# VISION-SJTU/UniDefense

Measured on AMD Instinct MI355X. Metric: images/sec fwd+bwd (256x256, EffNet-b4), higher is better.
Workload: dtype f32

## Files before the change

### include/unidefense_hip.h

```cpp
#ifndef UNIDEFENSE_HIP_H
#define UNIDEFENSE_HIP_H
#include <stdint.h>

#ifdef __cplusplus
extern "C" {
#endif

#define UD_EINVAL (-1000)

typedef void* ud_stream_t;

typedef struct {
    int N, Hin, Win, Cin, Hout, Wout, KH, KW, stride, pad_t, pad_l, transposed;
} ud_conv_geom;

typedef struct {
    const float* A; const float* B; float* C;
    int M, N, K;
    long lda, ldb, ldc;
    int a_mode, b_mode, out_mode, split_k;
    int batch; long strideA, strideB, strideC;
    ud_conv_geom g;
    double* stat_sum; double* stat_sumsq;
    int half_mask;
// ... 427 lines not shown
                          const uint32_t* skip_absmax, float* out, uint16_t* planes, long panel_stride, long plane_stride,
                          float* inv_scale, int G, int R, int C, uint32_t* absmax, ud_stream_t stream);
int ud_normbwd_sums(const void* x, const void* dy, const float* keep, float inv_keep, const ud_bn_ref* bn, int
    dy_is_dz, int G, int R, int C, double* s1, double* s2, double* s3, double* ws, int f16, ud_stream_t stream);
int ud_normbwd_apply(const void* x, const void* dy, const float* keep, float inv_keep, const ud_bn_ref* bn, int
    dy_is_dz, const double* s1, const double* s2, const double* s1_local, const double* s2_local, int G, int R,
    int C, void* dx, float* dgamma, float* dbeta, int f16, uint32_t* absmax, ud_stream_t stream);
int ud_normbwd_apply_planes(const float* x, const float* dy, const float* keep, float inv_keep, const ud_bn_ref* bn,
                            int dy_is_dz, const double* s1, const double* s2, const double* s1_local,
                            const double* s2_local, const double* energy, int G, int R, int C, uint16_t* planes,
                            long panel_stride, long plane_stride, float* inv_scale, float* dgamma, float* dbeta,
                            ud_stream_t stream);
int ud_pw_bwd_fused_ok(int CE, int CIN);
int ud_pw_bwd_set_form(int form);
long ud_pw_bwd_fused_grid(long M);
int ud_pw_bwd_fused(const float* e, const float* dz, const ud_bn_ref* bn, const double* s1, const double* s2,
                    const double* s1_local, const double* s2_local, const float* x, const float* w, const float* add, long M,
                    int CE, int CIN, float* dx, float* dw, float* part, float* dgamma, float* dbeta, ud_stream_t stream);
int ud_pj_bwd_fused_ok(int CE, int CO, int HW);
int ud_pj_fwd_fused_ok(int CE, int CO, int HW);
int ud_pj_fwd_fused(const float* d, const ud_bn_ref* bn, const float* s, const float* w, int N, int HW, int CE, int CO, float* p,
                    double* sum, double* sumsq, ud_stream_t stream);
long ud_pj_bwd_fused_grid(int N, int HW, int CE, int CO);
int ud_mb_eval_dw_ok(int Ci, int CE, int K, int stride);
long ud_mb_eval_dw_tiles(int Ho, int Wo, int stride);
int ud_mb_eval_dw(const float* x, const float* we, const ud_bn_ref* bn0, const float* wt, const ud_bn_ref* bn1, float* d, float* part,
                  int N, int H, int W, int Ci, int CE, int Ho, int Wo, int K, int stride, int pad_t, int pad_l, int out_act,
                  ud_stream_t stream);
int ud_mb_eval_dw_h_ok(int Ci, int CE, int K, int stride);
long ud_mb_eval_dw_h_tiles(int Ho, int Wo, int stride);
// ... 135 lines not shown
```

### unidefense_amd/csrc/pjbwd.hip

```cpp
#include "pw_common.h"

#include <type_traits>

namespace {

using namespace pw;

constexpr int NTH = 256;
constexpr int R = 32;

__device__ __forceinline__ void atomic_add_f64(double* p, double v) { unsafeAtomicAdd(p, v); }

template <int CE, int CO, int CC = CE> struct PjCfg {
    static_assert(CE % CC == 0 && CC % 8 == 0 && (CC % 16 == 0 || CC == CE) && CO % 8 == 0 && CO > 16 && CO <= 64, "thin project convs");
    static constexpr int CCP = (CC + 15) / 16 * 16;
    static constexpr int NCH = CE / CC;
    static constexpr int QT = CE / 4;
    static constexpr int Q = CC / 4;
    static constexpr int NIT = (R * Q + NTH - 1) / NTH;
    static constexpr int RI = (NIT * NTH + Q - 1) / Q;
    static constexpr int NBC = CCP / 16;
    static constexpr int NBW = (NBC + 3) / 4;
    static constexpr int CS = CCP * 2 + 16;
    static constexpr int CP = RI * CS;
// ... 656 lines not shown
            for (int c = tid; c < CC; c += NTH) atomic_add_f64(a.energy + c0 + c, eacc[c]);
        }
        acc = ud_wave_sum_d(acc);
        if (lane == 0) wsum[wave] = acc;
        __syncthreads();
        if (tid == 0) atomic_add_f64(a.dalpha + (blockIdx.x & 63), (wsum[0] + wsum[1]) + (wsum[2] + wsum[3]));
    }
}

template <int CE, int CO> struct PjFwdCfg {
    using B = PjCfg<CE, CO>;
    static constexpr int KD = (CE + 31) / 32 * 32;
    static constexpr int KS = KD / 32;
    static constexpr int CS = KD * 2 + 16;
    static constexpr int CP = B::RI * CS;
    static constexpr int LDS = 3 * CP + B::COEF + CE * 4 + 2 * 4 * 32 * 8;
};

struct PjFwdArgs {
    const float* d;
    const float* w;
    const float* s;
    float* p;
    double* sum;
    double* sumsq;
    const double* bsum;
    const double* bsumsq;
    const float* rmean;
    const float* rvar;
    const float* gamma;
    const float* beta;
    double inv_count;
    float eps;
    int act;
    int HW;
    long M;
    long tiles;
};

template <int CE, int CO>
__global__ __launch_bounds__(NTH, 2) void pj_fwd_kernel(PjFwdArgs a) {
    using CB = PjCfg<CE, CO>;
    using CF = PjFwdCfg<CE, CO>;
    static_assert(CO > 16 && CO <= 32, "two 16-column blocks: one (row block, column block) per wave");
    extern __shared__ __attribute__((aligned(16))) char L[];
    char* cimg = L;
    float* coef = reinterpret_cast<float*>(L + 3 * CF::CP);
    float* gate = coef + 4 * CE;
    double* wsum = reinterpret_cast<double*>(gate + CE);
    const lds_char* Lp = (const lds_char*)L;
    const int tid = threadIdx.x, lane = tid & 63;
    const int wave = __builtin_amdgcn_readfirstlane(tid >> 6);
    const int u = lane & 15, g = lane >> 4;
    const int mb = wave >> 1, nb = wave & 1;
    const bool swish = a.act == 1;

    if constexpr (CF::KD != CE) {
        for (int i = tid; i < 3 * CF::CP / 16; i += NTH) reinterpret_cast<u32x4*>(L)[i] = u32x4{0u, 0u, 0u, 0u};
    }
    const f32x4* d4 = reinterpret_cast<const f32x4*>(a.d);
    const long t0 = (long)blockIdx.x * a.tiles / gridDim.x, t1 = (long)(blockIdx.x + 1) * a.tiles / gridDim.x;
    f32x4 rd[CB::NIT];
    auto prefetch = [&](long tile_) {
        const long tile = min(tile_, a.tiles - 1);
        const f32x4* db = d4 + tile * (R * CB::Q);
#pragma unroll
        for (int it = 0; it < CB::NIT; ++it) {
            const int idx = tid + it * NTH;
            rd[it] = db[((it + 1) * NTH <= R * CB::Q || idx < R * CB::Q) ? idx : 0];
// ... 29 lines not shown
            cur_n = n;
            __syncthreads();
        }
#pragma unroll
        for (int it = 0; it < CB::NIT; ++it) {
            const int idx = tid + it * NTH;
            const int row = idx / CB::Q, q = idx - row * CB::Q;
            const f32x4 mu = c4[q], is = c4[CB::Q + q], ga = c4[2 * CB::Q + q], be = c4[3 * CB::Q + q], gt = g4[q];
            f32x4 cv;
#pragma unroll
            for (int k = 0; k < 4; ++k) cv[k] = act_sel(ga[k] * ((rd[it][k] - mu[k]) * is[k]) + be[k], swish) * gt[k];
            store_split4(cimg + row * CF::CS + q * 8, CF::CP, cv);
        }
        __syncthreads();
        prefetch(tile + 1);
        f32x4 acc = {0.f, 0.f, 0.f, 0.f};
        const lds_char* arow = Lp + (16 * mb + u) * CF::CS + g * 16;
#pragma unroll
        for (int ks = 0; ks < CF::KS; ++ks) acc = mma6(read_rows(arow + ks * 64, CF::CP), frag_of(wf[ks]), acc);
        float* po = a.p + (tile * R + 16 * mb + 4 * g) * CO + 16 * nb + u;
        float t1_ = 0.f, t2_ = 0.f;
#pragma unroll
        for (int r = 0; r < 4; ++r) {
            if (CO == 32 || 16 * nb + u < CO) po[r * CO] = acc[r];
            t1_ += acc[r];
            t2_ += acc[r] * acc[r];
        }
        s1 += (double)t1_;
        s2 += (double)t2_;
        __syncthreads();
    }
    if (a.sum) {
        s1 += __shfl_xor(s1, 16, 64); s1 += __shfl_xor(s1, 32, 64);
        s2 += __shfl_xor(s2, 16, 64); s2 += __shfl_xor(s2, 32, 64);
        if (g == 0) { wsum[wave * 16 + u] = s1; wsum[64 + wave * 16 + u] = s2; }
        __syncthreads();
        if (tid < CO) {
            const int nbb = tid >> 4, uu = tid & 15;
            atomic_add_f64(a.sum + tid, wsum[nbb * 16 + uu] + wsum[(2 + nbb) * 16 + uu]);
            atomic_add_f64(a.sumsq + tid, wsum[64 + nbb * 16 + uu] + wsum[64 + (2 + nbb) * 16 + uu]);
        }
    }
}

template <int CE, int CO>
int launch_f(const PjFwdArgs& a, int grid, hipStream_t s) {
    using CF = PjFwdCfg<CE, CO>;
    static_assert(CF::LDS <= 64 * 1024, "dynamic LDS within the default limit");
    hipLaunchKernelGGL((pj_fwd_kernel<CE, CO>), dim3((unsigned)grid), dim3(NTH), CF::LDS, s, a);
    return 0;
}

template <int CE, int CO, int CC, bool SE = false>
int launch_a(const PjArgs& a, int grid, hipStream_t s) {
    using CF = PjCfg<CE, CO, CC>;
    static_assert(CF::LDS_A <= 80 * 1024, "two workgroups per CU");
    static bool attr_set = false;
    if (!attr_set) {
        if (hipFuncSetAttribute(reinterpret_cast<const void*>(&pj_bwd_a_kernel<CE, CO, CC, SE>), hipFuncAttributeMaxDynamicSharedMemorySize,
                                CF::LDS_A) != hipSuccess)
            return UD_EINVAL;
        attr_set = true;
    }
// ... 48 lines not shown
               const float* dgamma, const float* dbeta) {
    return args_ok(d, dp, bn, s, w, N, HW, CE, CO) && ud_pj_bwd_fused_se_ok(CE, CO, HW) && dpool && s1 && s2 && dd &&
           !((dgamma || dbeta) && (!s1_local || !s2_local));
}
void fill_c(PjArgs& a, const float* dpool, float inv_hw, const double* s1, const double* s2, const double* s1_local,
            const double* s2_local, float* dd, float* dgamma, float* dbeta) {
    a.dpool = dpool; a.inv_hw = inv_hw; a.bs1 = s1; a.bs2 = s2; a.bs1l = s1_local; a.bs2l = s2_local; a.dd = dd; a.dgamma = dgamma;
    a.dbeta = dbeta;
}

}

extern "C" {

int ud_pj_bwd_fused_ok(int CE, int CO, int HW) { return (chunk_of(CE, CO) && HW >= R && HW % R == 0) ? 1 : 0; }
int ud_pj_fwd_fused_ok(int CE, int CO, int HW) { return (CO <= 32 && chunk_of(CE, CO) == CE && HW >= R && HW % R == 0) ? 1 : 0; }

int ud_pj_bwd_fused_se_ok(int CE, int CO, int HW) { return (ud_pj_bwd_fused_ok(CE, CO, HW) && CO != 24) ? 1 : 0; }

long ud_pj_bwd_fused_grid(int N, int HW, int CE, int CO) {
    const int cc = chunk_of(CE, CO);
    if (N < 1 || HW < R || HW % R || !cc) return UD_EINVAL;
    const long tiles = (long)N * HW / R, nch = CE / cc, per = 512 / nch;
    return nch * (tiles < per ? tiles : per);
}

int ud_pj_fwd_fused(const float* d, const ud_bn_ref* bn, const float* s, const float* w, int N, int HW, int CE, int CO, float* p,
                     double* sum, double* sumsq, ud_stream_t stream) {
    if (!d || !bn || (!bn->sum && !ud_bn_eval_form(bn)) || !s || !w || !p || N < 1 || !ud_pj_fwd_fused_ok(CE, CO, HW) || bn->G != 1 || !bn->gamma || !bn->beta || (!sum != !sumsq))
        return UD_EINVAL;
    PjFwdArgs a;
    a.d = d; a.w = w; a.s = s; a.p = p; a.sum = sum; a.sumsq = sumsq;
    a.bsum = bn->sum; a.bsumsq = bn->sumsq; a.rmean = bn->running_mean; a.rvar = bn->running_var; a.gamma = bn->gamma; a.beta = bn->beta;
    a.inv_count = bn->inv_count; a.eps = bn->eps; a.act = bn->act; a.HW = HW;
    a.M = (long)N * HW; a.tiles = a.M / R;
    const int grid = (int)ud_pj_bwd_fused_grid(N, HW, CE, CO);
    hipStream_t st = (hipStream_t)stream;
    const int rc = CO == 32 ? (CE == 144 ? launch_f<144, 32>(a, grid, st) : launch_f<192, 32>(a, grid, st))
                            : (CE == 48 ? launch_f<48, 24>(a, grid, st) : launch_f<24, 24>(a, grid, st));
    if (rc) return rc;
    UD_LAUNCH_CHECK();
    return 0;
}

int ud_pj_bwd_fused_a(const float* d, const float* dp, const ud_bn_ref* bn, const float* s, const float* w, int N, int HW, int CE, int CO,
                      float* dw, double* dgate, float* part, ud_stream_t stream) {
    if (!args_ok(d, dp, bn, s, w, N, HW, CE, CO) || !dw || !dgate || !part) return UD_EINVAL;
    hipStream_t st = (hipStream_t)stream;
    PjArgs a;
    fill(a, d, dp, bn, s, w, N, HW, CE, CO);
    a.part = part; a.dgate = dgate;
    const int grid = (int)ud_pj_bwd_fused_grid(N, HW, CE, CO);
    const int rc = CO == 32 ? (CE == 144 ? launch_a<144, 32, 144>(a, grid, st) : launch_a<192, 32, 192>(a, grid, st))
// ... 73 lines not shown
```

### unidefense_amd/csrc/pwbwd.hip

```cpp
#include "pw_common.h"

#include <type_traits>

namespace {

constexpr int NTH = 256;
constexpr int R = 32;

using namespace pw;

template <int CE, int CIN> struct PwCfg {
    static_assert(CE % 16 == 0 && CIN % 8 == 0 && CIN > 16 && CIN <= 32, "thin expand convs: 16 < CIN <= 32");
    static constexpr int KD = (CE + 31) / 32 * 32;
    static constexpr int KS = KD / 32;
    static constexpr int DYS = KD * 2 + 16;
    static constexpr int Q = CE / 4;
    static constexpr int NIT = (R * Q + NTH - 1) / NTH;
    static constexpr int RI = (NIT * NTH + Q - 1) / Q;
    static constexpr int DYP = RI * DYS;
    static constexpr int NB = 2;
    static constexpr int XS = NB * 32 + 16;
    static constexpr int XP = (NTH / (CIN / 4) + 1) * XS;
    static constexpr int XQ = CIN / 4;
    static constexpr int MB = CE / 16;
    static constexpr int NBW = (MB + 1) / 2;
    static constexpr int IMG = 3 * DYP + 3 * XP;
    static constexpr int LDS = IMG + 5 * CE * 4;
};

struct PwArgs {
    const float* e;
    const float* dz;
    const float* x;
    const float* w;
    const float* add;
    float* dx;
    float* part;
    const double* bsum;
    const double* bsumsq;
    const float* gamma;
// ... 2 lines not shown
    double inv_count;
    float eps;
    long M;
    long tiles;
};

template <int CE, int CIN, int D, int WPC>
__global__ __launch_bounds__(NTH, WPC) void pw_bwd_kernel(PwArgs a) {
    using CF = PwCfg<CE, CIN>;
    extern __shared__ __attribute__((aligned(16))) char L[];
    const lds_char* Lp = (const lds_char*)L;
    float* coef = reinterpret_cast<float*>(L + CF::IMG);
    const int tid = threadIdx.x, lane = tid & 63;
    const int wave = __builtin_amdgcn_readfirstlane(tid >> 6);
    const int u = lane & 15, g = lane >> 4;
    const int mb_d = wave >> 1, nbk = wave & 1;

    for (int i = tid; i < CF::IMG / 16; i += NTH) reinterpret_cast<u32x4*>(L)[i] = u32x4{0u, 0u, 0u, 0u};
    for (int c = tid; c < CE; c += NTH) {
        const double m = a.bsum[c] * a.inv_count;
        double v = a.bsumsq[c] * a.inv_count - m * m;
        if (v < 0.0) v = 0.0;
        const float is = rsqrtf((float)(v + (double)a.eps));
        coef[c] = (float)m;
        coef[CE + c] = is;
        coef[2 * CE + c] = a.gamma[c] * is;
        coef[3 * CE + c] = (float)a.s1[c] * (float)a.inv_count;
        coef[4 * CE + c] = (float)a.s2[c] * (float)a.inv_count;
    }

    u32x4 wf[CF::KS][3];
// ... 13 lines not shown
                uint32_t p0, p1, p2;
                split2(v[2 * h], v[2 * h + 1], p0, p1, p2);
                wf[ks][0][h] = p0; wf[ks][1][h] = p1; wf[ks][2][h] = p2;
            }
        }
    }

    f32x4 accw[CF::NBW];
#pragma unroll
    for (int i = 0; i < CF::NBW; ++i) accw[i] = f32x4{0.f, 0.f, 0.f, 0.f};

    const f32x4* dz4 = reinterpret_cast<const f32x4*>(a.dz);
    const f32x4* e4 = reinterpret_cast<const f32x4*>(a.e);
    const f32x4* x4 = reinterpret_cast<const f32x4*>(a.x);
    const long lim4 = a.M * CF::Q, limx = a.M * CF::XQ;
    f32x4 rdz[D][CF::NIT], re[D][CF::NIT], rx[D];
    float rav[D][4];
    const float* const add_src = a.add ? a.add : a.dx;
    const bool has_add = a.add != nullptr;
    const int dcol = 16 * nbk + u;
    auto prefetch = [&](auto slot_c, long tile_) {
        constexpr int S = decltype(slot_c)::value;
        const long tile = min(tile_, a.tiles - 1);
        const long b4 = tile * (R * CF::Q);
#pragma unroll
        for (int it = 0; it < CF::NIT; ++it) {
            const int idx = tid + it * NTH;
            long i = b4 + idx;
            i = (idx < R * CF::Q && i < lim4) ? i : 0;
            rdz[S][it] = dz4[i];
            re[S][it] = e4[i];
        }
        long ix = tile * (R * CF::XQ) + tid;
        ix = (tid < R * CF::XQ && ix < limx) ? ix : 0;
        rx[S] = x4[ix];
        const long row0 = tile * R + 16 * mb_d + 4 * g;
#pragma unroll
        for (int r = 0; r < 4; ++r) rav[S][r] = add_src[min(row0 + r, a.M - 1) * CIN + min(dcol, CIN - 1)];
    };

    const f32x4* c4 = reinterpret_cast<const f32x4*>(coef);
    auto step = [&](auto slot_c, long tile) {
        constexpr int S = decltype(slot_c)::value;
        {
            const long b4 = tile * (R * CF::Q);
#pragma unroll
            for (int it = 0; it < CF::NIT; ++it) {
                const int idx = tid + it * NTH;
                {
                    const int row = idx / CF::Q, q = idx - row * CF::Q;
                    const bool ok = b4 + idx < lim4;
                    const f32x4 mu = c4[q], is = c4[CF::Q + q], gi = c4[2 * CF::Q + q], t1 = c4[3 * CF::Q + q], t2 = c4[4 * CF::Q + q];
                    f32x4 o;
#pragma unroll
                    for (int k = 0; k < 4; ++k) {
                        const float xh = (re[S][it][k] - mu[k]) * is[k];
                        o[k] = ok ? gi[k] * (rdz[S][it][k] - t1[k] - xh * t2[k]) : 0.f;
                    }
                    uint32_t p0[2], p1[2], p2[2];
                    split2(o[0], o[1], p0[0], p1[0], p2[0]);
                    split2(o[2], o[3], p0[1], p1[1], p2[1]);
                    char* dst = L + row * CF::DYS + q * 8;
                    *reinterpret_cast<u32x2*>(dst) = u32x2{p0[0], p0[1]};
                    *reinterpret_cast<u32x2*>(dst + CF::DYP) = u32x2{p1[0], p1[1]};
                    *reinterpret_cast<u32x2*>(dst + 2 * CF::DYP) = u32x2{p2[0], p2[1]};
                }
            }
            {
                const int row = tid / CF::XQ, q = tid - row * CF::XQ;
                const bool ok = tile * (R * CF::XQ) + tid < limx;
                uint32_t p0[2], p1[2], p2[2];
                split2(ok ? rx[S][0] : 0.f, ok ? rx[S][1] : 0.f, p0[0], p1[0], p2[0]);
                split2(ok ? rx[S][2] : 0.f, ok ? rx[S][3] : 0.f, p0[1], p1[1], p2[1]);
                char* dst = L + 3 * CF::DYP + row * CF::XS + q * 8;
                *reinterpret_cast<u32x2*>(dst) = u32x2{p0[0], p0[1]};
                *reinterpret_cast<u32x2*>(dst + CF::XP) = u32x2{p1[0], p1[1]};
                *reinterpret_cast<u32x2*>(dst + 2 * CF::XP) = u32x2{p2[0], p2[1]};
            }
        }
        __syncthreads();
        float av[4];
#pragma unroll
        for (int r = 0; r < 4; ++r) av[r] = has_add ? rav[S][r] : 0.f;
        prefetch(slot_c, tile + (long)D * gridDim.x);

        {
            f32x4 acc = {0.f, 0.f, 0.f, 0.f};
            const int col = dcol;
            const long row0 = tile * R + 16 * mb_d + 4 * g;
            const lds_char* arow = Lp + (16 * mb_d + u) * CF::DYS + g * 16;
#pragma unroll
            for (int ks = 0; ks < CF::KS; ++ks) {
                bf16x8 af[3];
#pragma unroll
                for (int p = 0; p < 3; ++p)
                    af[p] = __builtin_bit_cast(bf16x8, *reinterpret_cast<const __attribute__((address_space(3))) s16x8*>(arow + p * CF::DYP + ks * 64));
                const bf16x8 b0 = __builtin_bit_cast(bf16x8, wf[ks][0]), b1 = __builtin_bit_cast(bf16x8, wf[ks][1]),
                             b2 = __builtin_bit_cast(bf16x8, wf[ks][2]);
                acc = __builtin_amdgcn_mfma_f32_16x16x32_bf16(af[2], b0, acc, 0, 0, 0);
                acc = __builtin_amdgcn_mfma_f32_16x16x32_bf16(af[0], b2, acc, 0, 0, 0);
                acc = __builtin_amdgcn_mfma_f32_16x16x32_bf16(af[1], b1, acc, 0, 0, 0);
                acc = __builtin_amdgcn_mfma_f32_16x16x32_bf16(af[1], b0, acc, 0, 0, 0);
                acc = __builtin_amdgcn_mfma_f32_16x16x32_bf16(af[0], b1, acc, 0, 0, 0);
                acc = __builtin_amdgcn_mfma_f32_16x16x32_bf16(af[0], b0, acc, 0, 0, 0);
            }
#pragma unroll
            for (int r = 0; r < 4; ++r)
                if (col < CIN && row0 + r < a.M) a.dx[(row0 + r) * CIN + col] = acc[r] + av[r];
        }
        {
            const int q = u >> 2, pp = u & 3;
            bf16x8 bf[3];
            const lds_char* xb = Lp + 3 * CF::DYP + (8 * g + q) * CF::XS + (16 * nbk + 4 * pp) * 2;
#pragma unroll
            for (int p = 0; p < 3; ++p) {
                const s16x4 lo = __builtin_amdgcn_ds_read_tr16_b64_v4i16((__attribute__((address_space(3))) s16x4*)(xb + p * CF::XP));
                const s16x4 hi = __builtin_amdgcn_ds_read_tr16_b64_v4i16((__attribute__((address_space(3))) s16x4*)(xb + p * CF::XP + 4 * CF::XS));
                bf[p] = __builtin_bit_cast(bf16x8, __builtin_shufflevector(lo, hi, 0, 1, 2, 3, 4, 5, 6, 7));
            }
            const lds_char* ab = Lp + (8 * g + q) * CF::DYS + 4 * pp * 2;
#pragma unroll
            for (int i = 0; i < CF::NBW; ++i) {
                const int mbk = min((wave >> 1) + 2 * i, CF::MB - 1);
                {
                    bf16x8 af[3];
#pragma unroll
                    for (int p = 0; p < 3; ++p) {
                        const lds_char* s = ab + p * CF::DYP + mbk * 32;
                        const s16x4 lo = __builtin_amdgcn_ds_read_tr16_b64_v4i16((__attribute__((address_space(3))) s16x4*)(s));
                        const s16x4 hi = __builtin_amdgcn_ds_read_tr16_b64_v4i16((__attribute__((address_space(3))) s16x4*)(s + 4 * CF::DYS));
                        af[p] = __builtin_bit_cast(bf16x8, __builtin_shufflevector(lo, hi, 0, 1, 2, 3, 4, 5, 6, 7));
                    }
                    f32x4 c = accw[i];
                    c = __builtin_amdgcn_mfma_f32_16x16x32_bf16(af[2], bf[0], c, 0, 0, 0);
                    c = __builtin_amdgcn_mfma_f32_16x16x32_bf16(af[0], bf[2], c, 0, 0, 0);
                    c = __builtin_amdgcn_mfma_f32_16x16x32_bf16(af[1], bf[1], c, 0, 0, 0);
                    c = __builtin_amdgcn_mfma_f32_16x16x32_bf16(af[1], bf[0], c, 0, 0, 0);
                    c = __builtin_amdgcn_mfma_f32_16x16x32_bf16(af[0], bf[1], c, 0, 0, 0);
                    c = __builtin_amdgcn_mfma_f32_16x16x32_bf16(af[0], bf[0], c, 0, 0, 0);
                    accw[i] = c;
                }
            }
        }
        __syncthreads();
    };

    using std::integral_constant;
    {
        long t = blockIdx.x;
        prefetch(integral_constant<int, 0>{}, t);
        if constexpr (D > 1) { t += gridDim.x; prefetch(integral_constant<int, 1>{}, t); }
        if constexpr (D > 2) { t += gridDim.x; prefetch(integral_constant<int, 2>{}, t); }
        if constexpr (D > 3) { t += gridDim.x; prefetch(integral_constant<int, 3>{}, t); }
    }
    __syncthreads();
    for (long tile = blockIdx.x;;) {
// ... 11 lines not shown
            tile += gridDim.x;
        }
        if constexpr (D > 3) {
            if (tile >= a.tiles) break;
            step(integral_constant<int, 3>{}, tile);
            tile += gridDim.x;
        }
    }

    {
        float* part = a.part + (long)blockIdx.x * (CE * CIN);
        const int col = 16 * nbk + u;
        if (col < CIN) {
#pragma unroll
            for (int i = 0; i < CF::NBW; ++i) {
                const int mbk = (wave >> 1) + 2 * i;
                if (mbk < CF::MB) {
#pragma unroll
                    for (int r = 0; r < 4; ++r) part[(16 * mbk + 4 * g + r) * CIN + col] = accw[i][r];
                }
            }
        }
    }
}

__global__ __launch_bounds__(256) void pw_bwd_fold_kernel(const float* __restrict__ part, int nparts, int numel, float* __restrict__ dw,
                                                          const double* __restrict__ s1l, const double* __restrict__ s2l, int CE,
                                                          float* __restrict__ dgamma, float* __restrict__ dbeta) {
    __shared__ float red[16][17];
    const int el = threadIdx.x & 15, grp = threadIdx.x >> 4;
    const int i = blockIdx.x * 16 + el;
// ... 12 lines not shown
        float t = red[0][el];
#pragma unroll
        for (int j = 1; j < 16; ++j) t += red[j][el];
        dw[i] = t;
    }
    const int c = blockIdx.x * 256 + threadIdx.x;
    if (c < CE) {
        if (dbeta) dbeta[c] = (float)s1l[c];
        if (dgamma) dgamma[c] = (float)s2l[c];
    }
}

template <int CE, int CIN, int D, int WPC>
int launch(const PwArgs& a, int grid, hipStream_t s) {
    using CF = PwCfg<CE, CIN>;
    static_assert(CF::LDS <= 64 * 1024, "dynamic LDS within the default limit");
    hipLaunchKernelGGL((pw_bwd_kernel<CE, CIN, D, WPC>), dim3((unsigned)grid), dim3(NTH), CF::LDS, s, a);
    return 0;
}

int g_pw_form = 0;

}

int pw::fold_launch(const float* part, int nparts, int numel, float* dw, const double* s1l, const double* s2l, int CE, float* dgamma,
                    float* dbeta, hipStream_t s) {
    hipLaunchKernelGGL(pw_bwd_fold_kernel, dim3((unsigned)ud_cdiv(numel, 16)), dim3(256), 0, s, part, nparts, numel, dw, s1l, s2l, CE,
                       dgamma, dbeta);
    UD_LAUNCH_CHECK();
    return 0;
}

extern "C" {

int ud_pw_bwd_set_form(int form) {
    if (form < 0 || form > 4) return UD_EINVAL;
    g_pw_form = form;
    return 0;
}

int ud_pw_bwd_fused_ok(int CE, int CIN) { return (CE == 144 && CIN == 24) || (CE == 192 && CIN == 32); }

long ud_pw_bwd_fused_grid(long M) {
    if (M < 1) return UD_EINVAL;
    const long tiles = (M + R - 1) / R;
    return tiles < 512 ? tiles : 512;
}

int ud_pw_bwd_fused(const float* e, const float* dz, const ud_bn_ref* bn, const double* s1, const double* s2, const double* s1_local,
                    const double* s2_local, const float* x, const float* w, const float* add, long M, int CE, int CIN, float* dx,
                    float* dw, float* part, float* dgamma, float* dbeta, ud_stream_t stream) {
    if (ud_bn_eval_form(bn)) return UD_EINVAL;
    if (!e || !dz || !bn || !s1 || !s2 || !x || !w || !dx || !dw || !part || M < 1 || !ud_pw_bwd_fused_ok(CE, CIN) || bn->G != 1 ||
        !bn->gamma)
        return UD_EINVAL;
    if ((dgamma || dbeta) && (!s1_local || !s2_local)) return UD_EINVAL;
    hipStream_t s = (hipStream_t)stream;
    PwArgs a;
    a.e = e; a.dz = dz; a.x = x; a.w = w; a.add = add; a.dx = dx; a.part = part;
    a.bsum = bn->sum; a.bsumsq = bn->sumsq; a.gamma = bn->gamma; a.s1 = s1; a.s2 = s2;
    a.inv_count = bn->inv_count; a.eps = bn->eps; a.M = M; a.tiles = (M + R - 1) / R;
    const int grid = (int)ud_pw_bwd_fused_grid(M);
    const int form = g_pw_form ? g_pw_form : 1;
    int rc;
    if (CE == 144)
        rc = form == 1 ? launch<144, 24, 1, 2>(a, grid, s) : form == 2 ? launch<144, 24, 2, 2>(a, grid, s)
           : form == 3 ? launch<144, 24, 3, 1>(a, grid, s) : launch<144, 24, 4, 1>(a, grid, s);
    else
        rc = form == 1 ? launch<192, 32, 1, 2>(a, grid, s) : form == 2 ? launch<192, 32, 2, 2>(a, grid, s)
           : form == 3 ? launch<192, 32, 3, 1>(a, grid, s) : launch<192, 32, 4, 1>(a, grid, s);
    if (rc) return rc;
    UD_LAUNCH_CHECK();
    return pw::fold_launch(part, grid, CE * CIN, dw, s1_local, s2_local, CE, dgamma, dbeta, s);
}

}
```

### unidefense_amd/kernels.py

```python
import ctypes as C
import math
import os

import torch

from . import lib as _lib
from .config import cfg as CFG
from .devmem import Scratch, ZeroPool
from .lib import ConvGeom, GemmDesc, GemmP3Desc

_call = _lib.call
_const, _rows = _lib.const, _lib.const_rows

GEMM_PROFILE = None


def _stream():
    return C.c_void_p(torch.cuda.current_stream().cuda_stream)


def _p(t):
    if t is None:
        return None
    return C.c_void_p(t.data_ptr())
# ... 3011 lines not shown


def expand_bwd_fused(e, dz, bn, sacc, sacc_local, x2, w2, add=None):
    _chk(e, dz, x2, w2)
    Ce, Cin = w2.shape
    M = x2.shape[0]
    assert e.numel() == M * Ce and dz.numel() == M * Ce and x2.is_contiguous() and w2.is_contiguous()
    loc = sacc if sacc_local is None else sacc_local
    dx = add if add is not None else torch.empty_like(x2)
    if add is not None:
        _chk(add)
        assert add.numel() == M * Cin
    dw = empty((Ce, Cin), x2)
    dg = empty((Ce,), x2)
    db = empty((Ce,), x2)
    grid = _lib.call("ud_pw_bwd_fused_grid", M)
    part = empty((grid, Ce * Cin), x2)
    _call("ud_pw_bwd_fused", _p(e), _p(dz), C.byref(bn.ref()), _pd(sacc), _pd(sacc, Ce), _pd(loc), _pd(loc, Ce), _p(x2), _p(w2),
          _p(add), M, Ce, Cin, _p(dx), _p(dw), _p(part), _p(dg), _p(db), _stream())
    return dx, dw, dg, db


def project_bwd_fused_ok(d, w2, HW):
    return (CFG.project_bwd_fused and d.dtype == torch.float32 and w2.dtype == torch.float32 and
            (CFG.project_bwd_fused_wide or w2.shape[0] != 56) and (CFG.project_fused_narrow or w2.shape[0] != 24) and
            _lib.call("ud_pj_bwd_fused_ok", int(w2.shape[1]), int(w2.shape[0]), int(HW)) == 1)


def project_fwd_fused_ok(d, w2, HW):
    return (project_bwd_fused_ok(d, w2, HW) and _lib.call("ud_pj_fwd_fused_ok", int(w2.shape[1]), int(w2.shape[0]), int(HW)) == 1)

# ... 467 lines not shown
```

### unidefense_amd/mbconv.py

```python
import collections
from types import SimpleNamespace

import torch

from . import kernels as K
from . import tape as T
from .config import cfg


FUSED, HALF, EVAL_NODE, OPERATORS = "fused", "half", "eval_node", "operators"
TrunkMode = collections.namedtuple("TrunkMode", "kind wt dp", defaults=(None,))


_DW_TILED = True


_DW_TILE_OVERRIDE = {}
_DW_BWD_FUSED_OVERRIDE = {}


def _dw_tile_policy(sf, k, stride, H, half):
    ov = _DW_TILE_OVERRIDE.get((bool(sf), k, stride, H, bool(half)))
    if ov is not None and _DW_TILED:
        return ov
# ... 37 lines not shown
    if ov is not None:
        return ov
    return True


_PJ_BN1_FOLD_OVERRIDE = {}
_PJ_BN1_FOLD_RULE = {(False, 2, 64, 144): True, (False, 1, 64, 192): True, (True, 2, 32, 192): True, (True, 1, 32, 336): True}


def _pj_bn1_fold_policy(sf, stride, Ho, Ce):
    key = (bool(sf), stride, Ho, Ce)
    ov = _PJ_BN1_FOLD_OVERRIDE.get(key)
    if ov is not None:
        return ov
    return _PJ_BN1_FOLD_RULE.get(key, False)


BlockGeom = collections.namedtuple(
    "BlockGeom", "N H W Cin M k stride pt pl Ho Wo HWo Mo Ce Co Cs We Wsr Wse Wp Wf sf alpha s_f s_i")


def block_geom(blk, x):
    sp = blk.spec
    N, H, W, Cin = x.shape
    Ho, Wo = T.conv_out_hw(H, W, sp.k, sp.stride, sp.pad)
    Ce, Co, Cs = sp.cexp, sp.cout, sp.cse
    sf = sp.sf_norm is not None
    dwm = blk._depthwise_conv
    s_f, s_i = T._fft_scales(H, sp.sf_norm) if sf else (None, None)
    return BlockGeom(N, H, W, Cin, N * H * W, sp.k, sp.stride, sp.pad[2], sp.pad[0], Ho, Wo, Ho * Wo, N * Ho * Wo, Ce, Co, Cs,
# ... 183 lines not shown
    b.c_pl = (d.dtype == torch.float32 and g.Ce % 32 == 0 and cfg.spectral_p2 != "off"
              and K.spectral_takes_planes(g.Mo, g.Co, g.Ce, g.Wp, want_stats=True))
    c_amax = None
    if b.c_pl:
        c_amax = K.colsum_bn_amax(d, b.bn1, g.N, g.HWo, b.pool, update=True)
    else:
        K.colsum_bn(d, b.bn1, g.N, g.HWo, b.pool, update=True)
    b.s1 = K.fc_fwd_d(b.pool, 1.0 / g.HWo, g.Wsr, blk._se_reduce.bias, g.N)
    b.s2 = K.fc_fwd(b.s1, g.Wse, blk._se_expand.bias, 1)
    return c_amax


def _fwd_project(b, c_amax, next_blk):
    g, x, blk, d, bn1, s2 = b.geo, b.x, b.blk, b.d, b.bn1, b.s2
    acc2 = K.zeros64(2 * g.Co, x)
    if not b.c_pl and K.project_fwd_fused_ok(d, g.Wp, g.HWo):
        p, b.pctx = K.project_fwd_fused(d, bn1, s2, g.Wp, g.N, g.HWo, stats=acc2)
        done = True
    elif b.c_pl:
        c = K.se_scale_bn_planes(d, bn1, s2, g.N, g.HWo, c_amax)
        (p, done), b.pctx = K.spectral_fwd(c, g.Wp, stats=acc2)
    elif (d.dtype == torch.float16 and g.Ce % 8 == 0 and K.spectral_takes_plane_half(g.Mo, g.Co, g.Ce)):
        c = K.se_scale_bn_plane_half(d, bn1, s2, g.N, g.HWo)
        (p, done), b.pctx = K.spectral_fwd(c, g.Wp, stats=acc2)
    else:
        c = K.se_scale_bn(d, bn1, s2, g.N, g.HWo, want_absmax=True)
        (p, done), b.pctx = K.spectral_fwd(c.view(g.Mo, g.Ce), g.Wp, stats=acc2, x_absmax=getattr(c, "_ud_absmax", None))
    if not done:
        K.colstats(p, acc2)
    b.dp.reduce(acc2)
    b.bn2 = _bn_of(blk._bn2, acc2, g.Mo * b.dp.world, 0)
# ... 169 lines not shown
        if b.t_bwd:
            gr.dx = K.dwtile_bwd_data(g_sp, wt, k, pt, pl, g.H, g.W, g_alpha, g_mode, add, stride=stride)
        else:
            gr.dx = K.dwconv_bwd_data_ex(g_sp, g_alpha, g_mode, wt, add, k, stride, pt, pl, g.H, g.W)
    if not skip_done:
        gr.dx = K.axpby(gr.dx, 1.0, dout, 1.0, out=gr.dx)


def _bwd_expand(b, tape, gr):
    g, x, blk, e, ectx, dz0, sb0, dout = b.geo, b.x, b.blk, b.e, b.ectx, gr.dz0, gr.sb0, gr.dout
    skip = blk.spec.skip
    if b.lazy_in is not None:
        b.lazy_in.backward(dz0, sb0, gr.is_dz)
        return None
    loc0 = b.dp.reduce(sb0, keep_local=True)
    thin = not gr.de_pl and e is not None and ectx.plans is None and K.expand_bwd_fused_ok(e, ectx.w, gr.is_dz)
    if thin:
        dx, dWe, dg0, db0 = _expand_dgrad(tape, skip, dout, x, lambda acc: K.expand_bwd_fused(e, dz0, b.bn0, sb0, loc0, ectx.x, ectx.w, add=acc))
    else:
        de2, de_amax, dg0, db0 = _normbwd_to_gemm(ectx, gr.de_pl, e, dz0, None, 1.0, b.bn0, gr.is_dz, 1, g.M, sb0, loc0)
    tape.add_param_grad(blk._bn0.weight, dg0)
    tape.add_param_grad(blk._bn0.bias, db0)
    if not thin:
        dx, dWe = _expand_dgrad(tape, skip, dout, x, lambda acc: K.spectral_bwd(ectx, de2, out=acc, dy_absmax=de_amax))
    tape.add_param_grad(blk._expand_conv.weight, dWe)
    return dx


def _half_forward(x, blk, g, wt, src_bn):
    bn1 = K.EvalBN(blk._bn1, 1)
    if g.We is not None:
# ... 99 lines not shown
            dx = K.axpby(dx, 1.0, dout, 1.0, out=dx)
    if probe is not None:
        probe(blk, "dx", dx)
    dx._ud_owned = True
    tape.add_grad(x, dx)


def eval_block_ok(blk, max_cin):
    sp = blk.spec
    return (sp.expand != 1 and sp.sf_norm is None and sp.cin <= max_cin and K.mb_eval_dw_ok(sp.cin, sp.cexp, sp.k, sp.stride))


def mbconv_eval(x, blk, wt):
    g = block_geom(blk, x)
    bn1 = K.EvalBN(blk._bn1, 1)
    pj = K.project_fwd_fused_ok(x, g.Wp, g.HWo)
    d, pool = K.mb_eval_dw(x, g.We, K.EvalBN(blk._bn0, 1), wt, bn1, g.k, g.stride, g.pt, g.pl, g.Ho, g.Wo, out_act=not pj)
    s1 = K.fc_fwd(pool, g.Wsr, blk._se_reduce.bias, 0)
    s2 = K.fc_fwd(s1, g.Wse, blk._se_expand.bias, 1)
    if pj:
        p, _ = K.project_fwd_fused(d, bn1, s2, g.Wp, g.N, g.HWo)
    else:
        p = K.gemm_nt(K.se_scale_fwd(d, s2).view(g.Mo, g.Ce), g.Wp)
    return K.residual_bn(p.view(g.N, g.Ho, g.Wo, g.Co), K.EvalBN(blk._bn2, 0), None, 1.0, x if blk.spec.skip else None, g.N, g.HWo)
```

Measured before the change: 1480.

## Extend fused project-forward and expand-backward kernels to 56-channel stages

```diff
diff --git a/include/unidefense_hip.h b/include/unidefense_hip.h
--- a/include/unidefense_hip.h
+++ b/include/unidefense_hip.h
@@ -465,6 +465,7 @@
 int ud_pw_bwd_fused_ok(int CE, int CIN);
 int ud_pw_bwd_set_form(int form);
 long ud_pw_bwd_fused_grid(long M);
+int ud_pw_bwd_fused_parts(long M, int CE, int CIN);
 int ud_pw_bwd_fused(const float* e, const float* dz, const ud_bn_ref* bn, const double* s1, const double* s2,
                     const double* s1_local, const double* s2_local, const float* x, const float* w, const float* add, long M,
                     int CE, int CIN, float* dx, float* dw, float* part, float* dgamma, float* dbeta, ud_stream_t stream);
diff --git a/unidefense_amd/csrc/pjbwd.hip b/unidefense_amd/csrc/pjbwd.hip
--- a/unidefense_amd/csrc/pjbwd.hip
+++ b/unidefense_amd/csrc/pjbwd.hip
@@ -694,7 +694,8 @@
     static constexpr int KS = KD / 32;
     static constexpr int CS = KD * 2 + 16;
     static constexpr int CP = B::RI * CS;
-    static constexpr int LDS = 3 * CP + B::COEF + CE * 4 + 2 * 4 * 32 * 8;
+    static constexpr int WS = CO > 32 ? 2 * 4 * 16 * 8 : 2 * 4 * 32 * 8;
+    static constexpr int LDS = 3 * CP + B::COEF + CE * 4 + WS;
 };
 
 struct PjFwdArgs {
@@ -722,7 +723,9 @@
 __global__ __launch_bounds__(NTH, 2) void pj_fwd_kernel(PjFwdArgs a) {
     using CB = PjCfg<CE, CO>;
     using CF = PjFwdCfg<CE, CO>;
-    static_assert(CO > 16 && CO <= 32, "two 16-column blocks: one (row block, column block) per wave");
+    static_assert(CO > 16 && CO <= 64, "two 16-column blocks: one (row block, column block) per wave; four: a wave owns a column block");
+    constexpr bool WIDE = CO > 32;
+    constexpr int NMB = WIDE ? 2 : 1;
     extern __shared__ __attribute__((aligned(16))) char L[];
     char* cimg = L;
     float* coef = reinterpret_cast<float*>(L + 3 * CF::CP);
@@ -732,7 +735,7 @@
     const int tid = threadIdx.x, lane = tid & 63;
     const int wave = __builtin_amdgcn_readfirstlane(tid >> 6);
     const int u = lane & 15, g = lane >> 4;
-    const int mb = wave >> 1, nb = wave & 1;
+    const int mb = WIDE ? 0 : wave >> 1, nb = WIDE ? wave : wave & 1;
     const bool swish = a.act == 1;
 
     if constexpr (CF::KD != CE) {
@@ -792,17 +795,26 @@
         }
         __syncthreads();
         prefetch(tile + 1);
-        f32x4 acc = {0.f, 0.f, 0.f, 0.f};
+        f32x4 acc[NMB];
+#pragma unroll
+        for (int i = 0; i < NMB; ++i) acc[i] = f32x4{0.f, 0.f, 0.f, 0.f};
         const lds_char* arow = Lp + (16 * mb + u) * CF::CS + g * 16;
 #pragma unroll
-        for (int ks = 0; ks < CF::KS; ++ks) acc = mma6(read_rows(arow + ks * 64, CF::CP), frag_of(wf[ks]), acc);
+        for (int ks = 0; ks < CF::KS; ++ks) {
+            const Frag3 b = frag_of(wf[ks]);
+#pragma unroll
+            for (int i = 0; i < NMB; ++i) acc[i] = mma6(read_rows(arow + i * 16 * CF::CS + ks * 64, CF::CP), b, acc[i]);
+        }
         float* po = a.p + (tile * R + 16 * mb + 4 * g) * CO + 16 * nb + u;
         float t1_ = 0.f, t2_ = 0.f;
 #pragma unroll
-        for (int r = 0; r < 4; ++r) {
-            if (CO == 32 || 16 * nb + u < CO) po[r * CO] = acc[r];
-            t1_ += acc[r];
-            t2_ += acc[r] * acc[r];
+        for (int i = 0; i < NMB; ++i) {
+#pragma unroll
+            for (int r = 0; r < 4; ++r) {
+                if (CO % 16 == 0 || 16 * nb + u < CO) po[(16 * i + r) * CO] = acc[i][r];
+                t1_ += acc[i][r];
+                t2_ += acc[i][r] * acc[i][r];
+            }
         }
         s1 += (double)t1_;
         s2 += (double)t2_;
@@ -815,8 +827,13 @@
         __syncthreads();
         if (tid < CO) {
             const int nbb = tid >> 4, uu = tid & 15;
-            atomic_add_f64(a.sum + tid, wsum[nbb * 16 + uu] + wsum[(2 + nbb) * 16 + uu]);
-            atomic_add_f64(a.sumsq + tid, wsum[64 + nbb * 16 + uu] + wsum[64 + (2 + nbb) * 16 + uu]);
+            if constexpr (WIDE) {
+                atomic_add_f64(a.sum + tid, wsum[nbb * 16 + uu]);
+                atomic_add_f64(a.sumsq + tid, wsum[64 + nbb * 16 + uu]);
+            } else {
+                atomic_add_f64(a.sum + tid, wsum[nbb * 16 + uu] + wsum[(2 + nbb) * 16 + uu]);
+                atomic_add_f64(a.sumsq + tid, wsum[64 + nbb * 16 + uu] + wsum[64 + (2 + nbb) * 16 + uu]);
+            }
         }
     }
 }
@@ -824,7 +841,16 @@
 template <int CE, int CO>
 int launch_f(const PjFwdArgs& a, int grid, hipStream_t s) {
     using CF = PjFwdCfg<CE, CO>;
-    static_assert(CF::LDS <= 64 * 1024, "dynamic LDS within the default limit");
+    static_assert(CF::LDS <= 80 * 1024, "two workgroups per CU");
+    if constexpr (CF::LDS > 64 * 1024) {
+        static bool attr_set = false;
+        if (!attr_set) {
+            if (hipFuncSetAttribute(reinterpret_cast<const void*>(&pj_fwd_kernel<CE, CO>), hipFuncAttributeMaxDynamicSharedMemorySize,
+                                    CF::LDS) != hipSuccess)
+                return UD_EINVAL;
+            attr_set = true;
+        }
+    }
     hipLaunchKernelGGL((pj_fwd_kernel<CE, CO>), dim3((unsigned)grid), dim3(NTH), CF::LDS, s, a);
     return 0;
 }
@@ -903,7 +929,10 @@
 extern "C" {
 
 int ud_pj_bwd_fused_ok(int CE, int CO, int HW) { return (chunk_of(CE, CO) && HW >= R && HW % R == 0) ? 1 : 0; }
-int ud_pj_fwd_fused_ok(int CE, int CO, int HW) { return (CO <= 32 && chunk_of(CE, CO) == CE && HW >= R && HW % R == 0) ? 1 : 0; }
+int ud_pj_fwd_fused_ok(int CE, int CO, int HW) {
+    const bool pair = (CO <= 32 && chunk_of(CE, CO) == CE) || (CO == 56 && (CE == 192 || CE == 336));
+    return (pair && HW >= R && HW % R == 0) ? 1 : 0;
+}
 
 int ud_pj_bwd_fused_se_ok(int CE, int CO, int HW) { return (ud_pj_bwd_fused_ok(CE, CO, HW) && CO != 24) ? 1 : 0; }
 
@@ -923,9 +952,10 @@
     a.bsum = bn->sum; a.bsumsq = bn->sumsq; a.rmean = bn->running_mean; a.rvar = bn->running_var; a.gamma = bn->gamma; a.beta = bn->beta;
     a.inv_count = bn->inv_count; a.eps = bn->eps; a.act = bn->act; a.HW = HW;
     a.M = (long)N * HW; a.tiles = a.M / R;
-    const int grid = (int)ud_pj_bwd_fused_grid(N, HW, CE, CO);
+    const int grid = (int)(a.tiles < 512 ? a.tiles : 512);
     hipStream_t st = (hipStream_t)stream;
     const int rc = CO == 32 ? (CE == 144 ? launch_f<144, 32>(a, grid, st) : launch_f<192, 32>(a, grid, st))
+                 : CO == 56 ? (CE == 336 ? launch_f<336, 56>(a, grid, st) : launch_f<192, 56>(a, grid, st))
                             : (CE == 48 ? launch_f<48, 24>(a, grid, st) : launch_f<24, 24>(a, grid, st));
     if (rc) return rc;
     UD_LAUNCH_CHECK();
diff --git a/unidefense_amd/csrc/pwbwd.hip b/unidefense_amd/csrc/pwbwd.hip
--- a/unidefense_amd/csrc/pwbwd.hip
+++ b/unidefense_amd/csrc/pwbwd.hip
@@ -10,7 +10,7 @@
 using namespace pw;
 
 template <int CE, int CIN> struct PwCfg {
-    static_assert(CE % 16 == 0 && CIN % 8 == 0 && CIN > 16 && CIN <= 32, "thin expand convs: 16 < CIN <= 32");
+    static_assert(CE % 16 == 0 && CIN % 8 == 0 && CIN > 16 && CIN <= 64, "thin expand convs: 16 < CIN <= 64");
     static constexpr int KD = (CE + 31) / 32 * 32;
     static constexpr int KS = KD / 32;
     static constexpr int DYS = KD * 2 + 16;
@@ -18,12 +18,15 @@
     static constexpr int NIT = (R * Q + NTH - 1) / NTH;
     static constexpr int RI = (NIT * NTH + Q - 1) / Q;
     static constexpr int DYP = RI * DYS;
-    static constexpr int NB = 2;
+    static constexpr int NB = CIN > 32 ? 4 : 2;
+    static constexpr bool WIDE = NB == 4;
+    static constexpr int NMB = WIDE ? 2 : 1;
     static constexpr int XS = NB * 32 + 16;
-    static constexpr int XP = (NTH / (CIN / 4) + 1) * XS;
     static constexpr int XQ = CIN / 4;
+    static constexpr int NITX = (R * XQ + NTH - 1) / NTH;
+    static constexpr int XP = (NITX * NTH / XQ + 1) * XS;
     static constexpr int MB = CE / 16;
-    static constexpr int NBW = (MB + 1) / 2;
+    static constexpr int NBW = WIDE ? MB : (MB + 1) / 2;
     static constexpr int IMG = 3 * DYP + 3 * XP;
     static constexpr int LDS = IMG + 5 * CE * 4;
 };
@@ -56,7 +59,7 @@
     const int tid = threadIdx.x, lane = tid & 63;
     const int wave = __builtin_amdgcn_readfirstlane(tid >> 6);
     const int u = lane & 15, g = lane >> 4;
-    const int mb_d = wave >> 1, nbk = wave & 1;
+    const int mb_d = CF::WIDE ? 0 : wave >> 1, nbk = CF::WIDE ? wave : wave & 1;
 
     for (int i = tid; i < CF::IMG / 16; i += NTH) reinterpret_cast<u32x4*>(L)[i] = u32x4{0u, 0u, 0u, 0u};
     for (int c = tid; c < CE; c += NTH) {
@@ -100,8 +103,8 @@
     const f32x4* e4 = reinterpret_cast<const f32x4*>(a.e);
     const f32x4* x4 = reinterpret_cast<const f32x4*>(a.x);
     const long lim4 = a.M * CF::Q, limx = a.M * CF::XQ;
-    f32x4 rdz[D][CF::NIT], re[D][CF::NIT], rx[D];
-    float rav[D][4];
+    f32x4 rdz[D][CF::NIT], re[D][CF::NIT], rx[D][CF::NITX];
+    float rav[D][4 * CF::NMB];
     const float* const add_src = a.add ? a.add : a.dx;
     const bool has_add = a.add != nullptr;
     const int dcol = 16 * nbk + u;
@@ -117,12 +120,18 @@
             rdz[S][it] = dz4[i];
             re[S][it] = e4[i];
         }
-        long ix = tile * (R * CF::XQ) + tid;
-        ix = (tid < R * CF::XQ && ix < limx) ? ix : 0;
-        rx[S] = x4[ix];
+#pragma unroll
+        for (int it = 0; it < CF::NITX; ++it) {
+            const int idx = tid + it * NTH;
+            long ix = tile * (R * CF::XQ) + idx;
+            ix = (idx < R * CF::XQ && ix < limx) ? ix : 0;
+            rx[S][it] = x4[ix];
+        }
         const long row0 = tile * R + 16 * mb_d + 4 * g;
 #pragma unroll
-        for (int r = 0; r < 4; ++r) rav[S][r] = add_src[min(row0 + r, a.M - 1) * CIN + min(dcol, CIN - 1)];
+        for (int i = 0; i < CF::NMB; ++i)
+#pragma unroll
+            for (int r = 0; r < 4; ++r) rav[S][4 * i + r] = add_src[min(row0 + 16 * i + r, a.M - 1) * CIN + min(dcol, CIN - 1)];
     };
 
     const f32x4* c4 = reinterpret_cast<const f32x4*>(coef);
@@ -152,12 +161,14 @@
                     *reinterpret_cast<u32x2*>(dst + 2 * CF::DYP) = u32x2{p2[0], p2[1]};
                 }
             }
-            {
-                const int row = tid / CF::XQ, q = tid - row * CF::XQ;
-                const bool ok = tile * (R * CF::XQ) + tid < limx;
+#pragma unroll
+            for (int it = 0; it < CF::NITX; ++it) {
+                const int idx = tid + it * NTH;
+                const int row = idx / CF::XQ, q = idx - row * CF::XQ;
+                const bool ok = tile * (R * CF::XQ) + idx < limx;
                 uint32_t p0[2], p1[2], p2[2];
-                split2(ok ? rx[S][0] : 0.f, ok ? rx[S][1] : 0.f, p0[0], p1[0], p2[0]);
-                split2(ok ? rx[S][2] : 0.f, ok ? rx[S][3] : 0.f, p0[1], p1[1], p2[1]);
+                split2(ok ? rx[S][it][0] : 0.f, ok ? rx[S][it][1] : 0.f, p0[0], p1[0], p2[0]);
+                split2(ok ? rx[S][it][2] : 0.f, ok ? rx[S][it][3] : 0.f, p0[1], p1[1], p2[1]);
                 char* dst = L + 3 * CF::DYP + row * CF::XS + q * 8;
                 *reinterpret_cast<u32x2*>(dst) = u32x2{p0[0], p0[1]};
                 *reinterpret_cast<u32x2*>(dst + CF::XP) = u32x2{p1[0], p1[1]};
@@ -165,34 +176,41 @@
             }
         }
         __syncthreads();
-        float av[4];
-#pragma unroll
-        for (int r = 0; r < 4; ++r) av[r] = has_add ? rav[S][r] : 0.f;
+        float av[4 * CF::NMB];
+#pragma unroll
+        for (int r = 0; r < 4 * CF::NMB; ++r) av[r] = has_add ? rav[S][r] : 0.f;
         prefetch(slot_c, tile + (long)D * gridDim.x);
 
         {
-            f32x4 acc = {0.f, 0.f, 0.f, 0.f};
+            f32x4 acc[CF::NMB];
+#pragma unroll
+            for (int i = 0; i < CF::NMB; ++i) acc[i] = f32x4{0.f, 0.f, 0.f, 0.f};
             const int col = dcol;
             const long row0 = tile * R + 16 * mb_d + 4 * g;
             const lds_char* arow = Lp + (16 * mb_d + u) * CF::DYS + g * 16;
 #pragma unroll
             for (int ks = 0; ks < CF::KS; ++ks) {
-                bf16x8 af[3];
-#pragma unroll
-                for (int p = 0; p < 3; ++p)
-                    af[p] = __builtin_bit_cast(bf16x8, *reinterpret_cast<const __attribute__((address_space(3))) s16x8*>(arow + p * CF::DYP + ks * 64));
                 const bf16x8 b0 = __builtin_bit_cast(bf16x8, wf[ks][0]), b1 = __builtin_bit_cast(bf16x8, wf[ks][1]),
                              b2 = __builtin_bit_cast(bf16x8, wf[ks][2]);
-                acc = __builtin_amdgcn_mfma_f32_16x16x32_bf16(af[2], b0, acc, 0, 0, 0);
-                acc = __builtin_amdgcn_mfma_f32_16x16x32_bf16(af[0], b2, acc, 0, 0, 0);
-                acc = __builtin_amdgcn_mfma_f32_16x16x32_bf16(af[1], b1, acc, 0, 0, 0);
-                acc = __builtin_amdgcn_mfma_f32_16x16x32_bf16(af[1], b0, acc, 0, 0, 0);
-                acc = __builtin_amdgcn_mfma_f32_16x16x32_bf16(af[0], b1, acc, 0, 0, 0);
-                acc = __builtin_amdgcn_mfma_f32_16x16x32_bf16(af[0], b0, acc, 0, 0, 0);
-            }
-#pragma unroll
-            for (int r = 0; r < 4; ++r)
-                if (col < CIN && row0 + r < a.M) a.dx[(row0 + r) * CIN + col] = acc[r] + av[r];
+#pragma unroll
+                for (int i = 0; i < CF::NMB; ++i) {
+                    bf16x8 af[3];
+#pragma unroll
+                    for (int p = 0; p < 3; ++p)
+                        af[p] = __builtin_bit_cast(bf16x8, *reinterpret_cast<const __attribute__((address_space(3))) s16x8*>(arow + i * 16 * CF::DYS + p * CF::DYP + ks * 64));
+                    acc[i] = __builtin_amdgcn_mfma_f32_16x16x32_bf16(af[2], b0, acc[i], 0, 0, 0);
+                    acc[i] = __builtin_amdgcn_mfma_f32_16x16x32_bf16(af[0], b2, acc[i], 0, 0, 0);
+                    acc[i] = __builtin_amdgcn_mfma_f32_16x16x32_bf16(af[1], b1, acc[i], 0, 0, 0);
+                    acc[i] = __builtin_amdgcn_mfma_f32_16x16x32_bf16(af[1], b0, acc[i], 0, 0, 0);
+                    acc[i] = __builtin_amdgcn_mfma_f32_16x16x32_bf16(af[0], b1, acc[i], 0, 0, 0);
+                    acc[i] = __builtin_amdgcn_mfma_f32_16x16x32_bf16(af[0], b0, acc[i], 0, 0, 0);
+                }
+            }
+#pragma unroll
+            for (int i = 0; i < CF::NMB; ++i)
+#pragma unroll
+                for (int r = 0; r < 4; ++r)
+                    if (col < CIN && row0 + 16 * i + r < a.M) a.dx[(row0 + 16 * i + r) * CIN + col] = acc[i][r] + av[4 * i + r];
         }
         {
             const int q = u >> 2, pp = u & 3;
@@ -205,27 +223,28 @@
                 bf[p] = __builtin_bit_cast(bf16x8, __builtin_shufflevector(lo, hi, 0, 1, 2, 3, 4, 5, 6, 7));
             }
             const lds_char* ab = Lp + (8 * g + q) * CF::DYS + 4 * pp * 2;
-#pragma unroll
-            for (int i = 0; i < CF::NBW; ++i) {
-                const int mbk = min((wave >> 1) + 2 * i, CF::MB - 1);
-                {
-                    bf16x8 af[3];
+            constexpr int GB = CF::WIDE ? 3 : 1;
+            static_assert(CF::NBW % GB == 0, "whole groups of row blocks");
+#pragma unroll
+            for (int i = 0; i < CF::NBW; i += GB) {
+                bf16x8 af[GB][3];
+#pragma unroll
+                for (int j = 0; j < GB; ++j) {
+                    const int mbk = CF::WIDE ? i + j : min((wave >> 1) + 2 * i, CF::MB - 1);
 #pragma unroll
                     for (int p = 0; p < 3; ++p) {
                         const lds_char* s = ab + p * CF::DYP + mbk * 32;
                         const s16x4 lo = __builtin_amdgcn_ds_read_tr16_b64_v4i16((__attribute__((address_space(3))) s16x4*)(s));
                         const s16x4 hi = __builtin_amdgcn_ds_read_tr16_b64_v4i16((__attribute__((address_space(3))) s16x4*)(s + 4 * CF::DYS));
-                        af[p] = __builtin_bit_cast(bf16x8, __builtin_shufflevector(lo, hi, 0, 1, 2, 3, 4, 5, 6, 7));
+                        af[j][p] = __builtin_bit_cast(bf16x8, __builtin_shufflevector(lo, hi, 0, 1, 2, 3, 4, 5, 6, 7));
                     }
-                    f32x4 c = accw[i];
-                    c = __builtin_amdgcn_mfma_f32_16x16x32_bf16(af[2], bf[0], c, 0, 0, 0);
-                    c = __builtin_amdgcn_mfma_f32_16x16x32_bf16(af[0], bf[2], c, 0, 0, 0);
-                    c = __builtin_amdgcn_mfma_f32_16x16x32_bf16(af[1], bf[1], c, 0, 0, 0);
-                    c = __builtin_amdgcn_mfma_f32_16x16x32_bf16(af[1], bf[0], c, 0, 0, 0);
-                    c = __builtin_amdgcn_mfma_f32_16x16x32_bf16(af[0], bf[1], c, 0, 0, 0);
-                    c = __builtin_amdgcn_mfma_f32_16x16x32_bf16(af[0], bf[0], c, 0, 0, 0);
-                    accw[i] = c;
                 }
+                constexpr int PA[6] = {2, 0, 1, 1, 0, 0}, PB[6] = {0, 2, 1, 0, 1, 0};
+#pragma unroll
+                for (int t = 0; t < 6; ++t)
+#pragma unroll
+                    for (int j = 0; j < GB; ++j)
+                        accw[i + j] = __builtin_amdgcn_mfma_f32_16x16x32_bf16(af[j][PA[t]], bf[PB[t]], accw[i + j], 0, 0, 0);
             }
         }
         __syncthreads();
@@ -267,7 +286,7 @@
         if (col < CIN) {
 #pragma unroll
             for (int i = 0; i < CF::NBW; ++i) {
-                const int mbk = (wave >> 1) + 2 * i;
+                const int mbk = CF::WIDE ? i : (wave >> 1) + 2 * i;
                 if (mbk < CF::MB) {
 #pragma unroll
                     for (int r = 0; r < 4; ++r) part[(16 * mbk + 4 * g + r) * CIN + col] = accw[i][r];
@@ -310,7 +329,16 @@
 template <int CE, int CIN, int D, int WPC>
 int launch(const PwArgs& a, int grid, hipStream_t s) {
     using CF = PwCfg<CE, CIN>;
-    static_assert(CF::LDS <= 64 * 1024, "dynamic LDS within the default limit");
+    static_assert(CF::LDS <= 160 * 1024 / WPC, "WPC workgroups per CU");
+    if constexpr (CF::LDS > 64 * 1024) {
+        static bool attr_set = false;
+        if (!attr_set) {
+            if (hipFuncSetAttribute(reinterpret_cast<const void*>(&pw_bwd_kernel<CE, CIN, D, WPC>), hipFuncAttributeMaxDynamicSharedMemorySize,
+                                    CF::LDS) != hipSuccess)
+                return UD_EINVAL;
+            attr_set = true;
+        }
+    }
     hipLaunchKernelGGL((pw_bwd_kernel<CE, CIN, D, WPC>), dim3((unsigned)grid), dim3(NTH), CF::LDS, s, a);
     return 0;
 }
@@ -335,12 +363,18 @@
     return 0;
 }
 
-int ud_pw_bwd_fused_ok(int CE, int CIN) { return (CE == 144 && CIN == 24) || (CE == 192 && CIN == 32); }
+int ud_pw_bwd_fused_ok(int CE, int CIN) { return (CE == 144 && CIN == 24) || (CE == 192 && CIN == 32) || (CE == 336 && CIN == 56); }
 
 long ud_pw_bwd_fused_grid(long M) {
     if (M < 1) return UD_EINVAL;
     const long tiles = (M + R - 1) / R;
     return tiles < 512 ? tiles : 512;
+}
+
+int ud_pw_bwd_fused_parts(long M, int CE, int CIN) {
+    if (M < 1 || !ud_pw_bwd_fused_ok(CE, CIN)) return UD_EINVAL;
+    const int g = (int)ud_pw_bwd_fused_grid(M);
+    return (CIN > 32 && g > 256) ? 256 : g;
 }
 
 int ud_pw_bwd_fused(const float* e, const float* dz, const ud_bn_ref* bn, const double* s1, const double* s2, const double* s1_local,
@@ -356,10 +390,12 @@
     a.e = e; a.dz = dz; a.x = x; a.w = w; a.add = add; a.dx = dx; a.part = part;
     a.bsum = bn->sum; a.bsumsq = bn->sumsq; a.gamma = bn->gamma; a.s1 = s1; a.s2 = s2;
     a.inv_count = bn->inv_count; a.eps = bn->eps; a.M = M; a.tiles = (M + R - 1) / R;
-    const int grid = (int)ud_pw_bwd_fused_grid(M);
+    const int grid = ud_pw_bwd_fused_parts(M, CE, CIN);
     const int form = g_pw_form ? g_pw_form : 1;
     int rc;
-    if (CE == 144)
+    if (CE == 336)
+        rc = launch<336, 56, 1, 1>(a, grid, s);
+    else if (CE == 144)
         rc = form == 1 ? launch<144, 24, 1, 2>(a, grid, s) : form == 2 ? launch<144, 24, 2, 2>(a, grid, s)
            : form == 3 ? launch<144, 24, 3, 1>(a, grid, s) : launch<144, 24, 4, 1>(a, grid, s);
     else
diff --git a/unidefense_amd/kernels.py b/unidefense_amd/kernels.py
--- a/unidefense_amd/kernels.py
+++ b/unidefense_amd/kernels.py
@@ -3049,7 +3049,7 @@
     dw = empty((Ce, Cin), x2)
     dg = empty((Ce,), x2)
     db = empty((Ce,), x2)
-    grid = _lib.call("ud_pw_bwd_fused_grid", M)
+    grid = _lib.call("ud_pw_bwd_fused_parts", M, Ce, Cin)
     part = empty((grid, Ce * Cin), x2)
     _call("ud_pw_bwd_fused", _p(e), _p(dz), C.byref(bn.ref()), _pd(sacc), _pd(sacc, Ce), _pd(loc), _pd(loc, Ce), _p(x2), _p(w2),
           _p(add), M, Ce, Cin, _p(dx), _p(dw), _p(part), _p(dg), _p(db), _stream())
diff --git a/unidefense_amd/mbconv.py b/unidefense_amd/mbconv.py
--- a/unidefense_amd/mbconv.py
+++ b/unidefense_amd/mbconv.py
@@ -75,6 +75,30 @@
     if ov is not None:
         return ov
     return _PJ_BN1_FOLD_RULE.get(key, False)
+
+
+_PJ_FWD_WIDE_OVERRIDE = {}
+_PJ_FWD_WIDE_RULE = {(True, 2, 32, 192): False, (True, 1, 32, 336): False}
+
+
+def _pj_fwd_wide_policy(sf, stride, Ho, Ce):
+    key = (bool(sf), stride, Ho, Ce)
+    ov = _PJ_FWD_WIDE_OVERRIDE.get(key)
+    if ov is not None:
+        return ov
+    return _PJ_FWD_WIDE_RULE.get(key, False)
+
+
+_PW_BWD_WIDE_OVERRIDE = {}
+_PW_BWD_WIDE_RULE = {(32, 336, 56): True}
+
+
+def _pw_bwd_wide_policy(H, Ce, Cin):
+    key = (H, Ce, Cin)
+    ov = _PW_BWD_WIDE_OVERRIDE.get(key)
+    if ov is not None:
+        return ov
+    return _PW_BWD_WIDE_RULE.get(key, False)
 
 
 BlockGeom = collections.namedtuple(
@@ -288,7 +312,7 @@
 def _fwd_project(b, c_amax, next_blk):
     g, x, blk, d, bn1, s2 = b.geo, b.x, b.blk, b.d, b.bn1, b.s2
     acc2 = K.zeros64(2 * g.Co, x)
-    if not b.c_pl and K.project_fwd_fused_ok(d, g.Wp, g.HWo):
+    if not b.c_pl and K.project_fwd_fused_ok(d, g.Wp, g.HWo) and (g.Co != 56 or _pj_fwd_wide_policy(g.sf, g.stride, g.Ho, g.Ce)):
         p, b.pctx = K.project_fwd_fused(d, bn1, s2, g.Wp, g.N, g.HWo, stats=acc2)
         done = True
     elif b.c_pl:
@@ -488,7 +512,8 @@
         b.lazy_in.backward(dz0, sb0, gr.is_dz)
         return None
     loc0 = b.dp.reduce(sb0, keep_local=True)
-    thin = not gr.de_pl and e is not None and ectx.plans is None and K.expand_bwd_fused_ok(e, ectx.w, gr.is_dz)
+    thin = (not gr.de_pl and e is not None and ectx.plans is None and K.expand_bwd_fused_ok(e, ectx.w, gr.is_dz)
+            and (g.Cin != 56 or _pw_bwd_wide_policy(g.H, g.Ce, g.Cin)))
     if thin:
         dx, dWe, dg0, db0 = _expand_dgrad(tape, skip, dout, x, lambda acc: K.expand_bwd_fused(e, dz0, b.bn0, sb0, loc0, ectx.x, ectx.w, add=acc))
     else:
@@ -618,7 +643,7 @@
 def mbconv_eval(x, blk, wt):
     g = block_geom(blk, x)
     bn1 = K.EvalBN(blk._bn1, 1)
-    pj = K.project_fwd_fused_ok(x, g.Wp, g.HWo)
+    pj = g.Co != 56 and K.project_fwd_fused_ok(x, g.Wp, g.HWo)
     d, pool = K.mb_eval_dw(x, g.We, K.EvalBN(blk._bn0, 1), wt, bn1, g.k, g.stride, g.pt, g.pl, g.Ho, g.Wo, out_act=not pj)
     s1 = K.fc_fwd(pool, g.Wsr, blk._se_reduce.bias, 0)
     s2 = K.fc_fwd(s1, g.Wse, blk._se_expand.bias, 1)
```

New measurement: 1487, median of 6. No clear change (+0.5%).
